# jarek1992/raytracer_project

Measured on AMD Instinct MI355X. Metric: Msamples/sec (rays·bounces), higher is better.
Workload: dtype f64

## Files before the change

raytracer_project_amd/csrc/zr_commit.cpp:

```cpp
#include "zr_host_internal.h"
#include "zr_flatten.h"

namespace {

template <class F>
int each_prim_array(zr_scene* s, Flattener& fl, F&& f) {
    int rc;
    if ((rc = f(s->d_spheres, fl.spheres, ZR_PRIM_SPHERE, ZR_SPHERE_DOUBLES)) || (rc = f(s->d_sphere_mat, fl.sphere_mat, ZR_PRIM_SPHERE, 1)) ||
        (rc = f(s->d_tri_v, fl.tri_v, ZR_PRIM_TRIANGLE, ZR_TRI_STRIDE)) || (rc = f(s->d_tri_s, fl.tri_s, ZR_PRIM_TRIANGLE, ZR_TRI_SHADE_DOUBLES)) ||
        (rc = f(s->d_cubes, fl.cubes, ZR_PRIM_CUBE, ZR_CUBE_DOUBLES)) || (rc = f(s->d_cube_mat, fl.cube_mat, ZR_PRIM_CUBE, 1)) ||
        (rc = f(s->d_pcubes, fl.pcubes, ZR_KIND_PCUBE, ZR_PCUBE_STRIDE)) || (rc = f(s->d_pcube_mat, fl.pcube_mat, ZR_KIND_PCUBE, 1)) ||
        (rc = f(s->d_media, fl.media, ZR_PRIM_MEDIUM, 1)) || (rc = f(s->d_wrapped, fl.wrapped, ZR_KIND_WRAPPED, 1))) return rc;
    return ZR_OK;
}

int commit_host(zr_scene* s, std::shared_ptr<const CommitPlan> plan, PhaseTimer& ph, CommitSummary& cs, std::shared_ptr<HostBuild>& staging) {
    auto hb = std::make_shared<HostBuild>();
    int rc = build_host_tree(*s, plan, ph, *hb);
    if (rc) return rc;
    Flattener& fl = *hb->fl;
    int up_rc = ZR_OK;
    std::string up_err;
    std::thread uploader;
    const int device = s->ctx ? s->ctx->device : 0;
// ... 233 lines not shown
    d.cubes = s->d_cubes.p; d.cube_mat = s->d_cube_mat.p;
    d.pcubes = s->d_pcubes.p; d.pcube_mat = s->d_pcube_mat.p;
    d.media = s->d_media.p; d.wrapped = s->d_wrapped.p; d.insts = s->d_insts.p; d.ops = s->d_ops.p;
    d.mats = s->d_mats.p; d.texs = s->d_texs.p; d.texels = s->d_texels.p;
    d.n_mats = (uint32_t)s->materials.size();
    d.mat_kinds = 0;
    for (const zr_material& m : s->materials) d.mat_kinds |= 1u << m.kind;
    d.root = cs.root;
    s->leaf_objects = 0;
    for (int k = 0; k < 8; k++) { d.leaf_cnt[k] = plan.cnt[k]; s->leaf_objects += plan.cnt[k]; }
    s->fused_ok = false;
    if (s->leaf_objects > 0 && s->leaf_objects <= ZR_FUSED_OBJECTS && plan.cnt[ZR_KIND_INSTANCE] == 0) {
        zr::FusedObjs fo{};
        auto take = [&](uint32_t kind, const double* d_src, size_t stride, size_t doubles) -> int {
            for (uint32_t i = 0; i < plan.cnt[kind]; i++) {
                fo.kind[fo.n] = kind; fo.index[fo.n] = i;
                HIP_OK(hipMemcpy(fo.rec[fo.n], d_src + (size_t)i * stride, doubles * sizeof(double), hipMemcpyDeviceToHost));
                fo.n++;
            }
            return ZR_OK;
        };
        if ((rc = take(ZR_PRIM_SPHERE, s->d_spheres.p, ZR_SPHERE_DOUBLES, ZR_SPHERE_DOUBLES)) || (rc = take(ZR_PRIM_TRIANGLE, s->d_tri_v.p, ZR_TRI_STRIDE, 9)) ||
            (rc = take(ZR_PRIM_CUBE, s->d_cubes.p, ZR_CUBE_DOUBLES, ZR_CUBE_DOUBLES)) || (rc = take(ZR_KIND_PCUBE, s->d_pcubes.p, ZR_PCUBE_STRIDE, ZR_PCUBE_STRIDE))) return rc;
        std::vector<zr::DMedium> hm(plan.cnt[ZR_PRIM_MEDIUM]);
        if (!hm.empty()) HIP_OK(hipMemcpy(hm.data(), s->d_media.p, hm.size() * sizeof(zr::DMedium), hipMemcpyDeviceToHost));
        for (uint32_t i = 0; i < hm.size(); i++) {
            if (hm[i].chain_count != 0) continue;
            fo.kind[fo.n] = ZR_PRIM_MEDIUM; fo.index[fo.n] = i;
            const bool sph = hm[i].btype == ZR_PRIM_SPHERE;
            HIP_OK(hipMemcpy(fo.rec[fo.n], sph ? s->d_spheres.p + (size_t)hm[i].bindex * ZR_SPHERE_DOUBLES : s->d_cubes.p + (size_t)hm[i].bindex * ZR_CUBE_DOUBLES, (sph ? ZR_SPHERE_DOUBLES : ZR_CUBE_DOUBLES) * sizeof(double), hipMemcpyDeviceToHost));
            fo.rec[fo.n][6] = hm[i].neg_inv_density;
            const uint64_t idb = hm[i].id, tb = hm[i].btype;
            std::memcpy(&fo.rec[fo.n][7], &idb, 8); std::memcpy(&fo.rec[fo.n][8], &tb, 8);
            fo.n++;
        }
        bool scaled = false;
        for (uint32_t i = 0; i < fo.n; i++) if (fo.kind[i] == ZR_KIND_PCUBE && fo.rec[i][15] != 0.0) scaled = true;
        s->fused = fo; s->fused_ok = !scaled;
    }
    {
        if (z[ZR_KIND_INSTANCE]) s->leaf_level = 3;
        else if (z[ZR_KIND_WRAPPED] || !cs.plain_media) s->leaf_level = 2;
        else if (z[ZR_PRIM_CUBE] || z[ZR_KIND_PCUBE] || z[ZR_PRIM_MEDIUM]) s->leaf_level = 1;
        else s->leaf_level = 0;
        const int force = (int)env_double("ZR_EXTEND_LEVEL", -1);
        if (force > s->leaf_level && force <= 3) s->leaf_level = force;
        bool lean = s->leaf_level == 0 && env_double("ZR_SHADE_LEAN", 1) != 0;
        for (const zr_material& m : s->materials) {
            if (m.kind != ZR_MAT_LAMBERTIAN && m.kind != ZR_MAT_METAL && m.kind != ZR_MAT_DIELECTRIC && m.kind != ZR_MAT_LIGHT) lean = false;
            if (m.bump_tex != ZR_NO_TEXTURE) lean = false;
            if (m.kind != ZR_MAT_DIELECTRIC && (m.tex >= s->textures.size() || s->textures[m.tex].kind != ZR_TEX_SOLID)) lean = false;
        }
        d.shade_lean = lean ? 1u : 0u;
        d.shade_escape = lean && env_double("ZR_SHADE_ESCAPE", 1) != 0 ? 1u : 0u;
    }
    s->stack_demand = cs.stack_demand;
    if (std::getenv("ZR_QUANT_STATS")) std::fprintf(stderr, "[zr] 4-wide tree: depth %d, worst-case traversal stack %u entries\n", cs.quad_depth, s->stack_demand);
    s->stats[0] = cs.n_pairs; s->stats[1] = (uint64_t)cs.max_depth; s->stats[2] = plan.objs.size();
    s->stats[3] = cs.n_pairs * sizeof(zr::NodePair) + cs.n_quads * sizeof(zr::NodeQ) + (z[ZR_PRIM_SPHERE] * ZR_SPHERE_DOUBLES + z[ZR_PRIM_TRIANGLE] * (ZR_TRI_STRIDE + ZR_TRI_SHADE_DOUBLES) + z[ZR_PRIM_CUBE] * ZR_CUBE_DOUBLES +
                   z[ZR_KIND_PCUBE] * ZR_PCUBE_STRIDE) * sizeof(double) + (z[ZR_PRIM_SPHERE] + z[ZR_PRIM_CUBE]) * sizeof(uint32_t) + s->texels.size();
    s->builder = cs.builder;
    if (std::getenv("ZR_COMMIT_HASH")) {
        (void)hipDeviceSynchronize();
        auto fnv = [](const void* dev, size_t bytes) -> unsigned long long {
            std::vector<unsigned char> h(bytes);
            unsigned long long x = 1469598103934665603ull;
            if (bytes && hipMemcpy(h.data(), dev, bytes, hipMemcpyDeviceToHost) == hipSuccess) for (unsigned char b : h) { x ^= b; x *= 1099511628211ull; }
            return x;
        };
        std::fprintf(stderr, "[zr] commit hash (%s): quads %016llx (%zu), pairs %016llx (%zu)\n", cs.builder, fnv(s->d_quads.p, cs.n_quads * sizeof(zr::NodeQ)), cs.n_quads,
                     fnv(s->d_nodes.p, cs.n_pairs * sizeof(zr::NodePair)), cs.n_pairs);
    }
    s->committed = true;
    if (s->borrowed) {
        s->spheres.drop(); s->sphere_mat.drop(); s->tri_v.drop(); s->tri_n.drop(); s->tri_mat.drop(); s->cubes.drop(); s->cube_mat.drop();
        s->media.drop(); s->ops.drop(); s->objects.drop(); s->texels.drop(); s->objects_set = false; s->borrowed = false; s->released = true;
    }
    return ZR_OK;
}

}

extern "C" {

zr_scene* zr_scene_create(zr_ctx* c) {
    if (!c) { fail(ZR_E_INVALID, "null context"); return nullptr; }
    zr_scene* s = new zr_scene();
    s->ctx = c; s->device = c->device;
    return s;
}
void zr_scene_destroy(zr_scene* s) {
    if (!s) return;
    (void)hipSetDevice(s->device);
    delete s;
}

enum { SET_SPHERES = 1, SET_TRIANGLES = 2, SET_CUBES = 4, SET_MEDIA = 8, SET_OPS = 16, SET_OBJECTS = 32, SET_ALL_GEOMETRY = 63 };
#define CHECK_SCENE(s) do { if (!(s)) return fail(ZR_E_INVALID, "null scene"); (s)->committed = false; } while (0)
#define GEOMETRY_SET(s, bit) do { if ((s)->released) { (s)->reset_mask |= (bit); if (((s)->reset_mask & SET_ALL_GEOMETRY) == SET_ALL_GEOMETRY) { (s)->released = false; (s)->reset_mask = 0; } } } while (0)

int zr_scene_set_spheres(zr_scene* s, const double* p, const uint32_t* mat, size_t n) {
    CHECK_SCENE(s);
    if (n && (!p || !mat)) return fail(ZR_E_INVALID, "null sphere arrays");
    s->spheres.copy(p, n * 4); s->sphere_mat.copy(mat, n);
    GEOMETRY_SET(s, SET_SPHERES);
    return ZR_OK;
}
// ... 127 lines not shown
```

raytracer_project_amd/csrc/zr_device.h:

```cpp
#pragma once

#include <hip/hip_runtime.h>
#include <stdint.h>

#include "../../include/zr_capi.h"
#include "../../include/zr_rng.h"

#include "zr_device_types.h"

namespace zr {

struct V3 { double x, y, z; };
__device__ __forceinline__ V3 mk(double x, double y, double z) { V3 r; r.x = x; r.y = y; r.z = z; return r; }
__device__ __forceinline__ V3 operator+(V3 a, V3 b) { return mk(a.x + b.x, a.y + b.y, a.z + b.z); }
__device__ __forceinline__ V3 operator-(V3 a, V3 b) { return mk(a.x - b.x, a.y - b.y, a.z - b.z); }
__device__ __forceinline__ V3 operator-(V3 a) { return mk(-a.x, -a.y, -a.z); }
__device__ __forceinline__ V3 operator*(V3 a, V3 b) { return mk(a.x * b.x, a.y * b.y, a.z * b.z); }
__device__ __forceinline__ V3 operator*(double t, V3 v) { return mk(t * v.x, t * v.y, t * v.z); }
__device__ __forceinline__ V3 operator*(V3 v, double t) { return mk(t * v.x, t * v.y, t * v.z); }
__device__ __forceinline__ V3 vdiv(V3 v, double t) { double r = 1 / t; return mk(r * v.x, r * v.y, r * v.z); }
__device__ __forceinline__ double dot(V3 a, V3 b) { return a.x * b.x + a.y * b.y + a.z * b.z; }
__device__ __forceinline__ V3 cross(V3 a, V3 b) { return mk(a.y * b.z - a.z * b.y, a.z * b.x - a.x * b.z, a.x * b.y - a.y * b.x); }
__device__ __forceinline__ double len2(V3 a) { return a.x * a.x + a.y * a.y + a.z * a.z; }
__device__ __forceinline__ double len(V3 a) { return sqrt(len2(a)); }
// ... 783 lines not shown
    em = mk(0, 0, 0);
    if (rec.mat >= sc.n_mats) return false;
    const zr_material& m = sc.mats[rec.mat];
    const uint32_t kind = m.kind;
    if (kind == ZR_MAT_LIGHT) { em = lean_color(sc, m.tex); return false; }
    V3 ruv = mk(0, 0, 0);
    if (kind == ZR_MAT_LAMBERTIAN || kind == ZR_MAT_METAL) ruv = random_unit_vector(g);
    V3 ud = mk(0, 0, 0);
    if (kind == ZR_MAT_METAL || kind == ZR_MAT_DIELECTRIC) ud = unit(rin.d);
    if (kind == ZR_MAT_LAMBERTIAN) {
        V3 dir = rec.n + ruv;
        if (fabs(dir.x) < 1e-8 && fabs(dir.y) < 1e-8 && fabs(dir.z) < 1e-8) dir = rec.n;
        out.o = rec.p + (rec.n * 0.0001);
        out.d = dir;
        att = lean_color(sc, m.tex);
        return true;
    }
    if (kind == ZR_MAT_METAL) {
        V3 refl = reflect(ud, rec.n);
        V3 dir = unit(refl + (m.param * ruv));
        out.o = rec.p + (0.0001 * rec.n);
        out.d = dir;
        att = lean_color(sc, m.tex);
        return dot(dir, rec.n) > 0;
    }
    if (kind == ZR_MAT_DIELECTRIC) {
        att = mk(m.tint[0], m.tint[1], m.tint[2]);
        double ri = rec.front ? (1.0 / m.param) : m.param;
        double ct = fmin(dot(-ud, rec.n), 1.0);
        double st = sqrt(1.0 - ct * ct);
        bool refl = ri * st > 1.0;
        if (!refl) {
            double r0 = (1 - ri) / (1 + ri);
            r0 = r0 * r0;
            double rf = r0 + (1 - r0) * pow5(1 - ct);
            refl = rf > g.next();
        }
        V3 dir;
        if (refl) dir = reflect(ud, rec.n);
        else {
            double c2 = fmin(dot(-ud, rec.n), 1.0);
            V3 perp = ri * (ud + c2 * rec.n);
            V3 par = (-sqrt(fabs(1.0 - len2(perp)))) * rec.n;
            dir = perp + par;
        }
        V3 off = (dot(dir, rec.n) > 0) ? (0.0001 * rec.n) : (-0.0001 * rec.n);
        out.o = rec.p + off;
        out.d = dir;
        return true;
    }
    return false;
}

__device__ inline V3 background(const DScene& sc, const DEnv& env, V3 rd) {
    if (env.mode == ZR_ENV_SOLID_COLOR) return mk(env.solid[0], env.solid[1], env.solid[2]);
    V3 ud = unit(rd);
    if (env.mode == ZR_ENV_HDR_MAP) {
        if (env.hdr_tex == ZR_NO_TEXTURE) return mk(0, 0, 0);
        V3 d = ud;
        double x1 = env.cy * d.x + env.sy * d.z;
        double z1 = -env.sy * d.x + env.cy * d.z;
        d = mk(x1, d.y, z1);
        double y2 = env.cp * d.y - env.sp * d.z;
        double z2 = env.sp * d.y + env.cp * d.z;
        d = mk(d.x, y2, z2);
        double x3 = env.cr * d.x - env.sr * d.y;
        double y3 = env.sr * d.x + env.cr * d.y;
        d = mk(x3, y3, d.z);
        const double PI = 3.14159265358979323846;
        const zr_texture& t = sc.texs[env.hdr_tex];
        if (t.kind == ZR_TEX_IMAGE_F32 && t.width > 0 && t.height > 0 && t.width <= 16384 && t.height <= 16384) {
            const float xf = (float)d.x, yf = (float)d.y, zf = (float)d.z;
            const float PIf = 3.14159265358979323846f;
            const float fi = (atan2f(zf, xf) + PIf) * (0.15915494309189535f * (float)t.width);
            const float fj = acosf(fminf(fmaxf(yf, -1.0f), 1.0f)) * (0.3183098861837907f * (float)t.height);
            const float ri = fi - floorf(fi), rj = fj - floorf(fj);
            const float guard = 0.02f;
            if (fabsf(yf) < 0.999f && ri > guard && ri < 1.0f - guard && rj > guard && rj < 1.0f - guard && fi > guard &&
                fi < (float)t.width - guard) {
                const int i = (int)fi, j = (int)fj;
                const float* px = (const float*)(sc.texels + t.texel_offset) + ((size_t)j * t.width + i) * 3;
                return mk((double)px[0], (double)px[1], (double)px[2]) * env.intensity;
            }
        }
        double phi = atan2(d.z, d.x) + PI;
        double theta = acos(clampd(d.y, -1.0, 1.0));
        return tex_value(sc, env.hdr_tex, phi / (2 * PI), theta / PI, mk(0, 0, 0)) * env.intensity;
    }
    V3 hor = mk(env.horizon[0], env.horizon[1], env.horizon[2]);
    V3 zen = mk(env.zenith[0], env.zenith[1], env.zenith[2]);
    V3 sun = mk(env.sun[0], env.sun[1], env.sun[2]);
    double a = ud.y;
    V3 sky;
    if (a > 0.0) sky = (1.0 - a) * hor + a * zen; else sky = hor * 0.1;
    V3 fin = (sky * env.sky_scale) * env.sky_exposure;
    double focus = dot(ud, sun);
    if (env.sun_on && focus > env.sun_thr) {
        double x = clampd((focus - env.sun_thr) / ((env.sun_thr + 0.0002) - env.sun_thr), 0.0, 1.0);
        double alpha = x * x * (3 - 2 * x);
        fin = fin + mk(env.sun_add[0], env.sun_add[1], env.sun_add[2]) * alpha;
    }
    return fin;
}

__device__ inline Ray camera_ray(const DCamera& cam, int i, int j, Rng& g) {
    double ox = g.next() - 0.5;
    double oy = g.next() - 0.5;
    V3 ps = ld3(cam.pixel00) + ((i + ox) * ld3(cam.du)) + ((j + oy) * ld3(cam.dv));
    V3 org = ld3(cam.center);
    if (cam.defocus) {
        double px, py;
        for (;;) {
            px = g.range(-1, 1);
            py = g.range(-1, 1);
            if (px * px + py * py + 0.0 * 0.0 < 1) break;
        }
        org = ld3(cam.center) + (px * ld3(cam.disk_u)) + (py * ld3(cam.disk_v));
    }
    Ray r; r.o = org; r.d = ps - org;
    return r;
}

}
```

raytracer_project_amd/csrc/zr_device_types.h:

```cpp
#pragma once
#include <stdint.h>
#include "../../include/zr_capi.h"

#define ZR_KIND_WRAPPED 4u
#define ZR_KIND_PCUBE 5u
#define ZR_KIND_INSTANCE 6u
#ifndef ZR_TRI_STRIDE
#define ZR_TRI_STRIDE 9
#endif
#define ZR_SPHERE_DOUBLES 4
#define ZR_CUBE_DOUBLES 6
#define ZR_TRI_SHADE_DOUBLES 20
#define ZR_STACK_DEPTH 48
#define ZR_MAX_CHAIN 8

namespace zr {

struct alignas(64) NodePair {
    float lo[2][3];
    float hi[2][3];
    uint32_t child[2];
    uint32_t meta[2];
};
static_assert(sizeof(NodePair) == 64, "NodePair must be 64 bytes");

#define ZR_PCUBE_STRIDE 16
#define ZR_REF_LEAF 0x80000000u
#define ZR_REF_EMPTY 0xFFFFFFFFu
struct alignas(64) NodeQ {
    float origin[3];
    float scale[3];
    uint32_t q[6];
    uint32_t ref[4];
};
static_assert(sizeof(NodeQ) == 64, "NodeQ must be 64 bytes");
struct NodeF {
    float lox[4], loy[4], loz[4], hix[4], hiy[4], hiz[4];
    uint32_t ref[4];
};

struct DMedium {
    uint32_t btype, bindex, chain_first, chain_count;
    uint32_t mat, id;
    double neg_inv_density;
};
struct DWrapped { uint32_t type, index, chain_first, chain_count; };
struct DInstance { uint32_t chain_first, chain_count, root , pad_ ; };

struct DScene {
    const NodePair* nodes;
    const NodeQ* quads;
    const double* spheres;
    const uint32_t* sphere_mat;
    const double* tri_v;
    const double* tri_s;
    const double* cubes;
    const uint32_t* cube_mat;
    const double* pcubes;
    const uint32_t* pcube_mat;
    const DMedium* media;
    const DWrapped* wrapped;
    const DInstance* insts;
    const zr_xform_op* ops;
    const zr_material* mats;
    const zr_texture* texs;
    const unsigned char* texels;
    uint32_t n_mats;
    uint32_t mat_kinds;
    uint32_t shade_lean;
    uint32_t leaf_cnt[8];
    NodeF root;
    uint32_t shade_escape;
};

struct DCamera {
    double center[3], pixel00[3], du[3], dv[3], disk_u[3], disk_v[3];
    int32_t W, H, spp, max_depth;
    int32_t defocus;
    int32_t pad_;
};

struct DEnv {
    uint32_t mode, hdr_tex;
    double solid[3];
    double cy, sy, cp, sp, cr, sr;
    double intensity;
    double sun[3];
    double horizon[3], zenith[3];
    double sky_scale, sky_exposure;
    double sun_thr;
    double sun_add[3];
    int32_t sun_on, pad_;
};

}
```

raytracer_project_amd/csrc/zr_stream.hip:

```cpp
#include "zr_device.h"
#include "zr_launch.h"

namespace zr {

#ifndef ST_EXT_WAVES
#define ST_EXT_WAVES 4
#endif
#ifndef ST_CHUNK
#define ST_CHUNK 256
#endif
#ifndef ST_SHADE_WAVES
#define ST_SHADE_WAVES 4
#endif
#ifndef ST_EXT_WAVES_LEAN
#define ST_EXT_WAVES_LEAN 6
#endif
#ifndef ST_EXT_WAVES_MID
#define ST_EXT_WAVES_MID 4
#endif
#ifndef ST_FETCH_MIN
#define ST_FETCH_MIN 16
#endif
#define ST_SHARDS 64
#ifndef ST_LDS_STACK
#define ST_LDS_STACK 12
#endif

enum { F_FIRST = 1u << 16, F_ACTIVE = 1u << 17, F_L0 = 1u << 18,
       F_LZERO = 1u << 19 , F_BONE = 1u << 20  };

struct SEntry { uint32_t node; float tn; };

enum { SF_RAY = 0, SF_HIT_T = 6, SF_HIT_KI = 7, SF_BETA = 8, SF_L = 11, SF_ATT0 = 14, SF_SUM = 17, SF_KEY = 20,
       SF_MA = 21 , SF_MB = 22 , SF_N = 24 };

enum { CTL_COMPACT = 4,
       CTL_SHARD0 = 16, CTL_STRIDE = 32,
       CTL_SH_UNITS = 0,
       CTL_SH_CHUNK = 8,
       CTL_SH_ACTIVE = 16 };

struct StreamBuf {
    double* pool;
    const uint32_t* pixels;
    double* samples;
    unsigned int* ctl;
    unsigned int* uctl;
    uint32_t P, spp, n_units, n_pix;
    uint32_t unit0;
    uint32_t unit_base;
    uint32_t unit_chunk;
    uint32_t shard_k0;
    uint32_t sample0;
    uint2* kend;
    unsigned char* cls;
    unsigned long long* cpart;
    __device__ __forceinline__ double* cell(int f, uint32_t slot) const { return pool + ((size_t)(slot >> 6) * SF_N + f) * 64 + (slot & 63u); }
    __device__ __forceinline__ double ld(int f, uint32_t slot) const { return *cell(f, slot); }
    __device__ __forceinline__ void st(int f, uint32_t slot, double v) const { *cell(f, slot) = v; }
    __device__ __forceinline__ uint2 ld2(int f, uint32_t slot) const { return *reinterpret_cast<const uint2*>(cell(f, slot)); }
    __device__ __forceinline__ void st2(int f, uint32_t slot, uint2 v) const { *reinterpret_cast<uint2*>(cell(f, slot)) = v; }
    __device__ __forceinline__ V3 ld3(int f, uint32_t slot) const { return mk(ld(f, slot), ld(f + 1, slot), ld(f + 2, slot)); }
    __device__ __forceinline__ void st3(int f, uint32_t slot, V3 v) const { st(f, slot, v.x); st(f + 1, slot, v.y); st(f + 2, slot, v.z); }
};

struct SlotAt {
    const char* base; uint32_t off;
    __device__ __forceinline__ const char* at(int f) const { return base + (off + (uint32_t)f * 512u); }
    __device__ __forceinline__ double ld(int f) const { return *reinterpret_cast<const double*>(at(f)); }
    __device__ __forceinline__ void st(int f, double v) const { *reinterpret_cast<double*>(const_cast<char*>(at(f))) = v; }
    __device__ __forceinline__ uint2 ld2(int f) const { return *reinterpret_cast<const uint2*>(at(f)); }
    __device__ __forceinline__ void st2(int f, uint2 v) const { *reinterpret_cast<uint2*>(const_cast<char*>(at(f))) = v; }
    __device__ __forceinline__ V3 ld3(int f) const { return mk(ld(f), ld(f + 1), ld(f + 2)); }
    __device__ __forceinline__ void st3(int f, V3 v) const { st(f, v.x); st(f + 1, v.y); st(f + 2, v.z); }
};
__device__ __forceinline__ SlotAt slot_at(const StreamBuf& B, uint32_t block, uint32_t src) {
    SlotAt a;
    a.base = reinterpret_cast<const char*>(B.pool) + (size_t)block * (size_t)(4 * SF_N * 512);
    a.off = (src >> 6) * (uint32_t)(SF_N * 512) + (src & 63u) * 8u;
    return a;
}


__host__ __device__ inline unsigned long long st_unit_of(uint32_t G, uint32_t unit_base, uint32_t shard, unsigned long long k) {
    if (G == 0) return (unsigned long long)unit_base + k * ST_SHARDS + shard;
    const uint32_t k32 = (uint32_t)k, q = k32 / G, r = k32 - q * G;
    const uint32_t pos = (shard & 7u) * (ST_SHARDS / 8u) + (shard >> 3);
    return ((unsigned long long)q * ST_SHARDS + pos) * G + r;
}
__host__ __device__ inline unsigned long long st_first_unit(uint32_t G, uint32_t g) {
    if (G == 0) return g;
    const uint32_t c = g >> 8;
    return st_unit_of(G, 0, c % ST_SHARDS, (unsigned long long)(c / ST_SHARDS) * 256u + (g & 255u));
}

__device__ inline void begin_sample(const StreamBuf& B, const DCamera& cam, uint64_t seed, const SlotAt& S, uint32_t unit, uint32_t& c_samp) {
    const uint32_t pix_i = unit / B.spp, sample = unit - pix_i * B.spp + B.sample0;
    const uint32_t pk = B.pixels[pix_i];
    const int px = (int)(pk & 0xFFFFu), py = (int)(pk >> 16);
    Rng g; g.key = zr_stream_key(seed, (uint64_t)py * (uint64_t)cam.W + (uint64_t)px, (uint64_t)sample); g.k = 0; g.bounce = 0;
    Ray r = camera_ray(cam, px, py, g);
    S.st3(SF_RAY, r.o); S.st3(SF_RAY + 3, r.d);
    S.st(SF_KEY, __longlong_as_double((long long)g.key));
    uint2 ma; ma.x = (uint32_t)g.k; ma.y = F_FIRST | F_ACTIVE;
    uint2 mb; mb.x = unit; mb.y = 0;
    S.st2(SF_MA, ma); S.st2(SF_MB, mb);
    c_samp++;
}

template <bool COUNT>
__global__ __launch_bounds__(256) void stream_init(StreamBuf B, DCamera cam, uint64_t seed, unsigned long long* __restrict__ gctr) {
    const uint32_t slot = blockIdx.x * 256 + threadIdx.x;
    if (slot >= B.P) return;
    uint32_t c_samp = 0;
    const unsigned long long u0 = st_first_unit(B.unit_chunk, B.unit0 + slot);
    const SlotAt S = slot_at(B, blockIdx.x, threadIdx.x);
    if (u0 < (unsigned long long)B.n_units) begin_sample(B, cam, seed, S, (uint32_t)u0, c_samp);
    else { uint2 z; z.x = 0; z.y = 0; S.st2(SF_MA, z); }
    if (COUNT && c_samp) atomicAdd(&gctr[CTR_SAMPLES], (unsigned long long)c_samp);
}

enum { X_IDLE = 0, X_NODE = 1, X_LEAF = 2 };
#define X_LEAF_BIT ZR_REF_LEAF

__device__ __forceinline__ void cswap(float& ta, uint32_t& ra, float& tb, uint32_t& rb) {
    const bool sw = tb < ta;
    const float t0 = sw ? tb : ta, t1 = sw ? ta : tb;
    const uint32_t r0 = sw ? rb : ra, r1 = sw ? ra : rb;
    ta = t0; tb = t1; ra = r0; rb = r1;
}

#ifndef ST_EXT_GROUP
#define ST_EXT_GROUP 1
#endif
template <bool COUNT, int LEVEL>
__global__ __launch_bounds__(64 * ST_EXT_GROUP, LEVEL >= 2 ? ST_EXT_WAVES : (LEVEL == 1 ? ST_EXT_WAVES_MID : ST_EXT_WAVES_LEAN)) void stream_extend(DScene sc, StreamBuf B, SEntry* __restrict__ overflow,
                                                                  uint32_t ovf_levels, unsigned long long* __restrict__ gctr) {
    __shared__ SEntry lstack[ST_EXT_GROUP * ST_LDS_STACK * 64];
    const int lane = threadIdx.x & 63;
    const uint32_t wave_id = blockIdx.x * ST_EXT_GROUP + (threadIdx.x >> 6);
    const int lbase = (int)(threadIdx.x >> 6) * ST_LDS_STACK * 64 + lane;
    const unsigned long long lt_mask = (1ull << lane) - 1ull;
    SEntry* gstack = overflow + (size_t)wave_id * ovf_levels * 64 + lane;
    const double INF = __builtin_huge_val();
    const float INFf = __builtin_huge_valf();
    const uint32_t NONE = 0xFFFFFFFFu;

    int st = X_IDLE;
    uint32_t slot = 0;
    Ray ray; ray.o = mk(0, 0, 0); ray.d = mk(0, 0, 1);
    float idx_ = 0, idy_ = 0, idz_ = 0;
    float cnx = 0, cny = 0, cnz = 0, cfx = 0, cfy = 0, cfz = 0;
    double tbest = INF;
    float tbest_f = INFf;
    uint32_t kbest = NONE, ibest = 0;
    uint32_t inst_cur = 0;
    uint32_t cur = 0;
    uint32_t pend_i = 0;
    int sp = 0;
// ... 193 lines not shown
                }
                bool h;
                if (LEVEL == 3 && lkind == ZR_KIND_INSTANCE) {
                    const DInstance in = sc.insts[prim];
                    ZR_PUSH(ZR_REF_LEAF | (7u << 28), -INFf)
                    ray = chain_ray(sc, in.chain_first, in.chain_count, ray);
                    ZR_RAY_CONSTANTS()
                    inst_cur = prim + 1u;
                    cur = in.pad_; pend_i = 0; st = X_NODE;
                } else if (LEVEL == 3 && lkind == 7u) {
                    ray.o = B.ld3(SF_RAY, slot); ray.d = B.ld3(SF_RAY + 3, slot);
                    ZR_RAY_CONSTANTS()
                    inst_cur = 0;
                    ZR_POP_NEXT()
                } else {
                if (LEVEL == 1) {
                    if (lkind == ZR_KIND_PCUBE) h = pcube_t(sc.pcubes + (size_t)prim * ZR_PCUBE_STRIDE, ray, 0.001, tbest, t);
                    else if (lkind == ZR_PRIM_CUBE) h = cube_t(sc.cubes + (size_t)prim * 6, ray, 0.001, tbest, t);
                    else h = medium_plain_t(sc, prim, ray, 0.001, tbest, g, t);
                } else h = object_t(sc, lkind, prim, ray, 0.001, tbest, g, t);
                if (h) { tbest = t; tbest_f = __double2float_ru(t); kbest = lkind; ibest = prim; }
                tested = true;
                }
            }
            if (tested) {
                pend_i++;
                if (pend_i > ((cur >> 24) & 0xFu)) { ZR_POP_NEXT() }
            }
        }
    }
    if (iter >= iter_cap && lane == 0) atomicAdd(&B.ctl[CTL_CAPPED], 1u);
#ifdef ZR_WAVE_PROFILE
    if (!COUNT && lane == 0) {
        atomicAdd(&gctr[CTR_PROF_WAVE_TICKS], wall_clock64() - t_begin); atomicAdd(&gctr[CTR_PROF_WAVES], 1ull);
        for (int k = 0; k < 3; k++) { atomicAdd(&gctr[CTR_PROF_EXECS + 2 * k], p_exec[k]); atomicAdd(&gctr[CTR_PROF_LANES + 2 * k], p_lanes[k]); }
        for (int k = 0; k < CTR_HIST_WORDS; k++) if (p_hist[threadIdx.x >> 6][k]) atomicAdd(&gctr[CTR_HIST + k], (unsigned long long)p_hist[threadIdx.x >> 6][k]);
    }
#endif
    if (COUNT) {
        atomicAdd(&gctr[CTR_SEGMENTS], (unsigned long long)c_seg);
        atomicAdd(&gctr[CTR_NODES], (unsigned long long)c_nodes);
        atomicAdd(&gctr[CTR_SPHERES], (unsigned long long)c_sph);
        atomicAdd(&gctr[CTR_TRIANGLES], (unsigned long long)c_tri);
        atomicAdd(&gctr[CTR_CUBES], (unsigned long long)c_cube);
        atomicAdd(&gctr[CTR_MEDIA], (unsigned long long)c_med);
        atomicAdd(&gctr[CTR_HITS], (unsigned long long)c_hits);
        if (lane == 0) for (int k = 0; k < 2; k++) { atomicAdd(&gctr[CTR_NODE_EXECS + 2 * k], s_exec[k]); atomicAdd(&gctr[CTR_NODE_LANES + 2 * k], s_lanes[k]); }
    }
}

#ifndef ST_SHADE_WAVES_LEAN
#define ST_SHADE_WAVES_LEAN 6
#endif
template <bool COUNT, int MODE, bool LEAN = false>
__global__ __launch_bounds__(256, LEAN ? ST_SHADE_WAVES_LEAN : ST_SHADE_WAVES) void stream_shade(DScene sc, DCamera cam, DEnv env, uint64_t seed, StreamBuf B,
                                                    unsigned long long* __restrict__ gctr) {
    const uint32_t slot0 = blockIdx.x * 256 + threadIdx.x;
    if (slot0 < ST_SHARDS) B.ctl[CTL_SHARD0 + CTL_STRIDE * slot0 + CTL_SH_CHUNK] = 0;
    __shared__ unsigned long long s_cnt[4];
    if (MODE != 0 && threadIdx.x < 4) s_cnt[threadIdx.x] = 0;
    __shared__ unsigned int wave_cls[4][8];
    __shared__ uint4 x_mk[256];
    __shared__ unsigned char x_src[256];
    uint32_t src;
    uint2 m, ki;
    {
        uint2 m0; m0.x = 0; m0.y = 0;
        uint2 k0; k0.x = 0xFFFFFFFFu; k0.y = 0;
        if (slot0 < B.P) { const SlotAt S0 = slot_at(B, blockIdx.x, threadIdx.x); m0 = S0.ld2(SF_MA); k0 = S0.ld2(SF_HIT_KI); }
        uint32_t cls = 7;
        if (m0.y & F_ACTIVE) {
            if (k0.x == 0xFFFFFFFFu) cls = 6;
            else {
                cls = 0;
                if (sc.mat_kinds & (sc.mat_kinds - 1u)) {
                    const uint32_t mat = object_material(sc, k0.x, k0.y);
                    cls = mat < sc.n_mats ? sc.mats[mat].kind : 5u;
                    if (cls > 5u) cls = 5u;
                }
            }
        }
        const int w = threadIdx.x >> 6, wl = threadIdx.x & 63;
        const unsigned long long below = (1ull << wl) - 1ull;
        unsigned int my_rank = 0;
#pragma unroll
        for (uint32_t c = 0; c < 8; c++) {
            const unsigned long long bm = __ballot(cls == c);
            if (wl == 0) wave_cls[w][c] = (unsigned int)__popcll(bm);
            if (cls == c) my_rank = (unsigned int)__popcll(bm & below);
        }
        __syncthreads();
        unsigned int base = 0;
        for (uint32_t c = 0; c < 8; c++)
            for (int k = 0; k < 4; k++)
                if (c < cls || (c == cls && k < w)) base += wave_cls[k][c];
        uint4 mk4; mk4.x = m0.x; mk4.y = m0.y; mk4.z = k0.x; mk4.w = k0.y;
        x_mk[base + my_rank] = mk4;
        x_src[base + my_rank] = (unsigned char)threadIdx.x;
        __syncthreads();
        mk4 = x_mk[threadIdx.x];
        src = x_src[threadIdx.x];
        m.x = mk4.x; m.y = mk4.y; ki.x = mk4.z; ki.y = mk4.w;
    }
    const SlotAt S = slot_at(B, blockIdx.x, src);
    bool active_after = false, want_unit = false;
    uint32_t c_samp = 0, c_seg2 = 0, c_hit2 = 0, c_esc = 0, c_esc_nodes = 0, c_seen = 0; unsigned long long c_draws = 0;
// ... 94 lines not shown
                                if (g.next() > p) stop = true; else beta = beta * (1 / p);
                            }
                        }
                    }
                    if (!stop) { b_inner++; if (b_inner >= depth_inner) stop = true; }
                    if (stop) {
                        if (!have_L) L = load_L();
                        if (MODE == 2) { const double luma = 0.2126 * len(L); if (luma > 2.0) L = L * (2.0 / luma); }
                        contrib = S.ld3(SF_ATT0) * L; ended = true;
                    } else if (esc) {
                        att0_now = S.ld3(SF_ATT0); beta_now = beta;
                        if (have_L) { L_now = L; have_L_now = true; }
                    } else {
                        if (have_L) { S.st3(SF_L, L); keep_lzero = 0; }
                        S.st3(SF_BETA, beta);
                    }
                }
                if (!ended && esc) {
                    escaped = true; miss_first = false;
                    ray = nr;
                    if (COUNT) { c_esc++; c_esc_nodes += esc_nodes; }
                } else if (!ended) {
                    S.st3(SF_RAY, nr.o); S.st3(SF_RAY + 3, nr.d);
                    if (has_add) S.st3(SF_SUM, add_now);
                    m.x = (uint32_t)g.k;
                    m.y = (g.bounce & 0xFFu) | ((uint32_t)b_inner << 8) | F_ACTIVE | (first ? (has_add ? F_L0 : 0u) : (m.y & F_L0)) |
                          (first ? (F_LZERO | F_BONE) : keep_lzero);
                    S.st2(SF_MA, m);
                    active_after = true;
                }
            }
            if (ESC && (ki.x == NONE || escaped)) ZR_MISS_STAGE()
#undef ZR_MISS_STAGE
            if (ended) {
                V3 rad = contrib;
                if (has_add) rad = add_now + rad;
                else if (MODE != 2 && !first && (m.y & F_L0)) rad = S.ld3(SF_SUM) + rad;
                const uint2 mb = mb_now;
                const uint32_t unit = mb.x;
                if (MODE != 2 || !no_output) {
                    double* pp = B.samples + (size_t)unit * 3;
                    pp[0] = rad.x; pp[1] = rad.y; pp[2] = rad.z;
                }
                if (MODE == 1) { uint2 ke; ke.x = (uint32_t)g.k; ke.y = g.bounce; B.kend[unit] = ke; }
                if (MODE == 2 && !no_output) B.cls[unit] = (unsigned char)mb.y;
                if (COUNT) {
                    if (MODE != 2) c_draws += g.k;
                    else if (!(first && ki.x == NONE)) c_draws += g.k - B.kend[unit].x;
                }
                want_unit = true;
            }
        }
    }
    {
        const unsigned long long wm = __ballot(want_unit);
        if (wm != 0ull) {
            const uint32_t shard = blockIdx.x % ST_SHARDS;
            const int wl = threadIdx.x & 63;
            uint32_t k0 = 0;
            if (wl == (int)__builtin_ctzll(wm)) k0 = atomicAdd(&B.uctl[CTL_STRIDE * shard + CTL_SH_UNITS], (unsigned int)__popcll(wm));
            k0 = __shfl(k0, (int)__builtin_ctzll(wm), 64);
            if (want_unit) {
                const unsigned long long k = (unsigned long long)k0 + (unsigned long long)__popcll(wm & ((1ull << wl) - 1ull));
                const unsigned long long u = st_unit_of(B.unit_chunk, B.unit_base, shard, (unsigned long long)B.shard_k0 + k);
                if (u < (unsigned long long)B.n_units) { begin_sample(B, cam, seed, S, (uint32_t)u, c_samp); active_after = true; }
                else { uint2 z; z.x = 0; z.y = 0; S.st2(SF_MA, z); }
            }
        }
    }
    const unsigned long long am = __ballot(active_after);
    if ((threadIdx.x & 63) == 0 && am != 0ull) atomicAdd(&B.ctl[CTL_SHARD0 + CTL_STRIDE * (blockIdx.x % ST_SHARDS) + CTL_SH_ACTIVE], (unsigned int)__popcll(am));
    if (COUNT && MODE == 0) {
        if (c_samp) atomicAdd(&gctr[CTR_SAMPLES], (unsigned long long)c_samp);
        if (c_draws) atomicAdd(&gctr[CTR_DRAWS], c_draws);
        if (c_seen) atomicAdd(&gctr[CTR_SHADE_LANES], (unsigned long long)c_seen);
        if (c_esc) {
            atomicAdd(&gctr[CTR_SEGMENTS], (unsigned long long)c_esc); atomicAdd(&gctr[CTR_ESCAPED], (unsigned long long)c_esc);
            atomicAdd(&gctr[CTR_NODES], (unsigned long long)c_esc_nodes);
        }
    }
    if (MODE != 0) {
        if (c_samp) atomicAdd(&s_cnt[0], (unsigned long long)c_samp);
        if (c_seg2) atomicAdd(&s_cnt[1], (unsigned long long)c_seg2);
        if (c_hit2) atomicAdd(&s_cnt[2], (unsigned long long)c_hit2);
        if (c_draws) atomicAdd(&s_cnt[3], c_draws);
        __syncthreads();
        if (threadIdx.x < 4 && s_cnt[threadIdx.x]) B.cpart[(size_t)blockIdx.x * 4 + threadIdx.x] += s_cnt[threadIdx.x];
    }
}

#ifndef ST_FUSED_CHUNK
#define ST_FUSED_CHUNK 256
#endif
#ifndef ST_FUSED_WAVES
#define ST_FUSED_WAVES 2
#endif
struct FusedBuf {
    const uint32_t* pixels; double* samples; unsigned int* uctl;
    uint32_t spp, n_units;
    uint32_t sample0;
    uint32_t chunk_lo, chunk_hi;
};
__device__ __forceinline__ bool medium_rec_t(const double* q, const Ray& r, double tmin, double tmax, const Rng& g, double& t) {
    double t1, t2;
    const double inf = __builtin_huge_val();
    const uint32_t btype = (uint32_t)__double_as_longlong(q[8]);
    if (btype == ZR_PRIM_SPHERE) {
        if (!sphere_t(q, r, -inf, inf, t1)) return false;
        if (!sphere_t(q, r, t1 + 0.0001, inf, t2)) return false;
    } else {
        if (!cube_t(q, r, -inf, inf, t1)) return false;
        if (!cube_t(q, r, t1 + 0.0001, inf, t2)) return false;
    }
    if (t1 < tmin) t1 = tmin;
    if (t2 > tmax) t2 = tmax;
    if (t1 >= t2) return false;
    if (t1 < 0) t1 = 0;
    const double rl = len(r.d);
    const double inside = (t2 - t1) * rl;
// ... 266 lines not shown
    uint2 ma; ma.x = 0; ma.y = 0;
    if (slot < n) {
        B.st3(SF_RAY, slot, ld3(rays + (size_t)slot * 6)); B.st3(SF_RAY + 3, slot, ld3(rays + (size_t)slot * 6 + 3));
        B.st(SF_KEY, slot, __longlong_as_double((long long)zr_stream_key(seed, pixel, (uint64_t)slot)));
        ma.y = (bounce & 0xFFu) | F_ACTIVE;
    }
    B.st2(SF_MA, slot, ma);
}

__global__ __launch_bounds__(256) void stream_hits_out(DScene sc, StreamBuf B, uint32_t n, zr_hit* __restrict__ out) {
    const uint32_t slot = blockIdx.x * 256 + threadIdx.x;
    if (slot >= n) return;
    const uint2 ki = B.ld2(SF_HIT_KI, slot);
    zr_hit o;
    if (ki.x != 0xFFFFFFFFu) {
        Ray r; r.o = B.ld3(SF_RAY, slot); r.d = B.ld3(SF_RAY + 3, slot);
        Rec rec;
        object_rec(sc, ki.x, ki.y, r, B.ld(SF_HIT_T, slot), rec, true);
        o.p[0] = rec.p.x; o.p[1] = rec.p.y; o.p[2] = rec.p.z;
        o.normal[0] = rec.n.x; o.normal[1] = rec.n.y; o.normal[2] = rec.n.z;
        o.tangent[0] = rec.tan.x; o.tangent[1] = rec.tan.y; o.tangent[2] = rec.tan.z;
        o.bitangent[0] = rec.bit.x; o.bitangent[1] = rec.bit.y; o.bitangent[2] = rec.bit.z;
        o.t = rec.t; o.u = rec.u; o.v = rec.v; o.mat = rec.mat; o.front_face = rec.front ? 1u : 0u;
    } else {
        for (int c = 0; c < 3; c++) { o.p[c] = 0; o.normal[c] = 0; o.tangent[c] = 0; o.bitangent[c] = 0; }
        o.t = 0; o.u = 0; o.v = 0; o.mat = 0xFFFFFFFFu; o.front_face = 0;
    }
    out[slot] = o;
}

size_t stream_ctl_words() { return CTL_SHARD0 + CTL_STRIDE * ST_SHARDS; }
uint32_t stream_overflow_levels(uint32_t stack_demand) { return stack_demand > ST_LDS_STACK ? stack_demand - ST_LDS_STACK : 1u; }
size_t stream_overflow_bytes(int blocks, uint32_t levels) { return (size_t)blocks * levels * 64 * sizeof(SEntry); }

int stream_extend_blocks() {
    int dev = 0, cus = 256, per_cu = 2;
    if (hipGetDevice(&dev) == hipSuccess) {
        hipDeviceProp_t p;
        if (hipGetDeviceProperties(&p, dev) == hipSuccess) cus = p.multiProcessorCount;
    }
    int lean = 0;
    if (hipOccupancyMaxActiveBlocksPerMultiprocessor(&per_cu, stream_extend<false, 2>, 64 * ST_EXT_GROUP, 0) != hipSuccess || per_cu < 1) per_cu = 2;
    if (hipOccupancyMaxActiveBlocksPerMultiprocessor(&lean, stream_extend<false, 0>, 64 * ST_EXT_GROUP, 0) == hipSuccess && lean > per_cu) per_cu = lean;
    if (std::getenv("ZR_COMMIT_STATS")) std::fprintf(stderr, "[zr] EXTEND workgroups per CU: %d (lean build %d) x %d waves\n", per_cu, lean, ST_EXT_GROUP);
    return cus * per_cu * ST_EXT_GROUP;
}

size_t stream_pool_bytes(uint32_t P) { return ((size_t)(P + 63) / 64) * SF_N * 64 * sizeof(double); }

static StreamBuf make_buf(void* pool, uint32_t P, uint32_t spp, uint32_t n_units, uint32_t n_pix, const uint32_t* pixels, double* samples,
                          unsigned int* ctl, unsigned int* uctl, uint32_t unit0, uint32_t unit_base) {
    StreamBuf B;
    B.pool = (double*)pool; B.pixels = pixels; B.samples = samples; B.ctl = ctl; B.uctl = uctl;
    B.P = P; B.spp = spp; B.n_units = n_units; B.n_pix = n_pix; B.unit0 = unit0; B.unit_base = unit_base; B.unit_chunk = 0; B.shard_k0 = 0; B.sample0 = 0;
    B.kend = nullptr; B.cls = nullptr; B.cpart = nullptr;
    return B;
}

template <bool COUNT>
static void launch_extend(const DScene& sc, const StreamBuf& B, void* overflow, uint32_t ovf_levels, int blocks, unsigned long long* gctr, int level, hipStream_t st) {
    const dim3 grid((blocks + ST_EXT_GROUP - 1) / ST_EXT_GROUP), group(64 * ST_EXT_GROUP);
    if (level >= 3) hipLaunchKernelGGL((stream_extend<COUNT, 3>), grid, group, 0, st, sc, B, (SEntry*)overflow, ovf_levels, gctr);
    else if (level == 2) hipLaunchKernelGGL((stream_extend<COUNT, 2>), grid, group, 0, st, sc, B, (SEntry*)overflow, ovf_levels, gctr);
    else if (level == 1) hipLaunchKernelGGL((stream_extend<COUNT, 1>), grid, group, 0, st, sc, B, (SEntry*)overflow, ovf_levels, gctr);
    else hipLaunchKernelGGL((stream_extend<COUNT, 0>), grid, group, 0, st, sc, B, (SEntry*)overflow, ovf_levels, gctr);
}

hipError_t stream_render(const DScene& sc, const StreamJob& job, int leaf_level) {
    const StreamFrame& F = job.frame; const StreamContext& X = job.ctx; const StreamHooks& H = job.hooks;
    const DCamera& cam = *F.cam; const DEnv& env = *F.env;
    const uint32_t P = job.pool.P, unit_chunk = job.pool.unit_chunk, n_pix = F.n_pix;
    const int mode = job.split.mode;
    const uint32_t n_units = n_pix * F.spp;
    const size_t W = stream_ctl_words();
    int K = X.n_pools < 1 ? 1 : (X.n_pools > ST_MAX_POOLS ? ST_MAX_POOLS : X.n_pools);
    while (K > 1 && P / K < 64u * 1024u) K--;
    const uint32_t pool_round = unit_chunk ? ST_SHARDS * 256u : 64u;
    if (unit_chunk && P % pool_round != 0) return hipErrorInvalidValue;
    while (K > 1 && P / K < pool_round) K--;
    StreamBuf Q[ST_MAX_POOLS];
    void* ov[ST_MAX_POOLS];
    unsigned int* uctl = X.ctl + (size_t)ST_MAX_POOLS * W;
    const unsigned int* h_units = X.h_active + (size_t)ST_MAX_POOLS * W;
    {
        uint32_t first = 0;
        unsigned char* base = (unsigned char*)job.pool.slots;
        for (int k = 0; k < K; k++) {
            uint32_t Pk = k == K - 1 ? P - first : (P / K + pool_round - 1) / pool_round * pool_round;
            Q[k] = make_buf(base, Pk, F.spp, n_units, n_pix, F.pixels, F.samples, X.ctl + (size_t)k * W, uctl, first, P);
            Q[k].unit_chunk = unit_chunk; Q[k].shard_k0 = unit_chunk ? P / ST_SHARDS : 0u; Q[k].sample0 = F.sample0;
            Q[k].kend = (uint2*)job.split.kend; Q[k].cls = (unsigned char*)job.split.cls;
            Q[k].cpart = job.split.cpart ? job.split.cpart + ((size_t)first / 256 + (size_t)k) * 4 : nullptr;
            ov[k] = (unsigned char*)X.overflow + (size_t)k * stream_overflow_bytes(X.extend_blocks, X.ovf_levels);
            base += stream_pool_bytes(Pk);
            first += Pk;
        }
    }
    hipError_t e;
    hipStream_t stream = X.streams[0];
    if ((e = hipMemsetAsync(X.ctl, 0, (ST_MAX_POOLS + 1) * W * sizeof(unsigned int), stream)) != hipSuccess) return e;
    const size_t cpart_blocks = (size_t)P / 256 + ST_MAX_POOLS + 1;
    if (job.split.cpart && (e = hipMemsetAsync(job.split.cpart, 0, cpart_blocks * 4 * sizeof(unsigned long long), stream)) != hipSuccess) return e;
    auto init = [&](const StreamBuf& B, hipStream_t st) {
        if (H.timer) H.timer->begin(st, 0);
        if (F.count) hipLaunchKernelGGL(stream_init<true>, dim3((B.P + 255) / 256), dim3(256), 0, st, B, cam, F.seed, X.gctr);
        else hipLaunchKernelGGL(stream_init<false>, dim3((B.P + 255) / 256), dim3(256), 0, st, B, cam, F.seed, X.gctr);
        if (H.timer) H.timer->end(st, 0);
    };
    auto extend = [&](const StreamBuf& B, void* o, hipStream_t st) {
        const int eb = (int)((B.P + 63) / 64 < (uint32_t)X.extend_blocks ? (B.P + 63) / 64 : (uint32_t)X.extend_blocks);
        if (H.timer) H.timer->begin(st, 1);
        if (F.count) launch_extend<true>(sc, B, o, X.ovf_levels, eb, X.gctr, leaf_level, st); else launch_extend<false>(sc, B, o, X.ovf_levels, eb, X.gctr, leaf_level, st);
        if (H.timer) H.timer->end(st, 1);
    };
    static const unsigned shade_pad = std::getenv("ZR_SHADE_LDS_PAD") ? (unsigned)std::atoi(std::getenv("ZR_SHADE_LDS_PAD")) : 0u;
    auto shade = [&](const StreamBuf& B, hipStream_t st) {
        if (H.timer) H.timer->begin(st, 2);
        const dim3 sg((B.P + 255) / 256), sb(256);
        if (sc.shade_lean && mode == 0) {
            if (F.count) hipLaunchKernelGGL((stream_shade<true, 0, true>), sg, sb, 0, st, sc, cam, env, F.seed, B, X.gctr);
            else hipLaunchKernelGGL((stream_shade<false, 0, true>), sg, sb, shade_pad, st, sc, cam, env, F.seed, B, X.gctr);
        }
        else if (shade_pad && mode == 0 && !F.count) hipLaunchKernelGGL((stream_shade<false, 0>), sg, sb, shade_pad, st, sc, cam, env, F.seed, B, X.gctr);
        else if (mode == 1) hipLaunchKernelGGL((stream_shade<true, 1>), sg, sb, 0, st, sc, cam, env, F.seed, B, X.gctr);
        else if (mode == 2) hipLaunchKernelGGL((stream_shade<true, 2>), sg, sb, 0, st, sc, cam, env, F.seed, B, X.gctr);
        else if (F.count) hipLaunchKernelGGL((stream_shade<true, 0>), sg, sb, 0, st, sc, cam, env, F.seed, B, X.gctr);
        else hipLaunchKernelGGL((stream_shade<false, 0>), sg, sb, 0, st, sc, cam, env, F.seed, B, X.gctr);
        if (H.timer) H.timer->end(st, 2);
    };
    init(Q[0], stream);
    for (int k = 1; k < K; k++) {
        extend(Q[k - 1], ov[k - 1], X.streams[k - 1]);
        if ((e = hipEventRecord(X.event, X.streams[k - 1])) != hipSuccess) return e;
        if ((e = hipStreamWaitEvent(X.streams[k], X.event, 0)) != hipSuccess) return e;
        init(Q[k], X.streams[k]);
        shade(Q[k - 1], X.streams[k - 1]);
    }
    int rounds = K > 1 ? 1 : 0;
    int check_every = H.progress ? 2 : 8;
    bool cancelled = false, drained = false, capped = false;
    for (;;) {
        for (int r = 0; r < check_every; r++) {
            for (int k = K - 1; k >= 0; k--) { extend(Q[k], ov[k], X.streams[k]); shade(Q[k], X.streams[k]); }
// ... 147 lines not shown
```

Baseline: 6956.

## Regenerate camera samples in lean shade and resolve provably escaping rays directly

In the lean shade kernel (MODE 0), a fresh camera sample is now tested with ray_escapes against the scene root when it is generated. If the ray provably misses all geometry, its background colour is written straight to the sample buffer and another unit is fetched in a loop, so such rays skip a full extend/shade round trip through the stream pool. Kernel arguments are reloaded from the kernarg segment pointer, presumably to limit register pressure. The change adds extra divergence and atomics per wave. regen_max defaults to 0, which leaves the loop unbounded, and the escape level now defaults to 2, so the new path runs by default.

```diff
diff --git a/raytracer_project_amd/csrc/zr_commit.cpp b/raytracer_project_amd/csrc/zr_commit.cpp
--- a/raytracer_project_amd/csrc/zr_commit.cpp
+++ b/raytracer_project_amd/csrc/zr_commit.cpp
@@ -309,7 +309,9 @@
             if (m.kind != ZR_MAT_DIELECTRIC && (m.tex >= s->textures.size() || s->textures[m.tex].kind != ZR_TEX_SOLID)) lean = false;
         }
         d.shade_lean = lean ? 1u : 0u;
-        d.shade_escape = lean && env_double("ZR_SHADE_ESCAPE", 1) != 0 ? 1u : 0u;
+        const double esc_level = env_double("ZR_SHADE_ESCAPE", 2), regen_max = env_double("ZR_SHADE_REGEN_MAX", ZR_SHADE_REGEN_MAX_DEFAULT);
+        d.shade_escape = (uint16_t)(lean && esc_level >= 1 ? (esc_level >= 2 ? 2 : 1) : 0);
+        d.regen_max = (uint16_t)(regen_max >= 1 ? std::min(regen_max, 65535.0) : 0);
     }
     s->stack_demand = cs.stack_demand;
     if (std::getenv("ZR_QUANT_STATS")) std::fprintf(stderr, "[zr] 4-wide tree: depth %d, worst-case traversal stack %u entries\n", cs.quad_depth, s->stack_demand);
diff --git a/raytracer_project_amd/csrc/zr_device.h b/raytracer_project_amd/csrc/zr_device.h
--- a/raytracer_project_amd/csrc/zr_device.h
+++ b/raytracer_project_amd/csrc/zr_device.h
@@ -859,9 +859,14 @@
     return false;
 }
 
-__device__ inline V3 background(const DScene& sc, const DEnv& env, V3 rd) {
+template <bool DIRECT = false>
+__device__ inline V3 background(const DScene& sc, const DEnv& env, V3 rd, bool* direct_ok = nullptr) {
     if (env.mode == ZR_ENV_SOLID_COLOR) return mk(env.solid[0], env.solid[1], env.solid[2]);
-    V3 ud = unit(rd);
+    V3 ud;
+    if (DIRECT) {
+        const double l = sqrt(__builtin_fma(rd.z, rd.z, __builtin_fma(rd.x, rd.x, rd.y * rd.y)));
+        ud = l < 1e-8 ? mk(0, 0, 0) : vdiv(rd, l);
+    } else ud = unit(rd);
     if (env.mode == ZR_ENV_HDR_MAP) {
         if (env.hdr_tex == ZR_NO_TEXTURE) return mk(0, 0, 0);
         V3 d = ud;
@@ -890,6 +895,7 @@
                 return mk((double)px[0], (double)px[1], (double)px[2]) * env.intensity;
             }
         }
+        if (DIRECT) { *direct_ok = false; return mk(0, 0, 0); }
         double phi = atan2(d.z, d.x) + PI;
         double theta = acos(clampd(d.y, -1.0, 1.0));
         return tex_value(sc, env.hdr_tex, phi / (2 * PI), theta / PI, mk(0, 0, 0)) * env.intensity;
@@ -899,9 +905,12 @@
     V3 sun = mk(env.sun[0], env.sun[1], env.sun[2]);
     double a = ud.y;
     V3 sky;
-    if (a > 0.0) sky = (1.0 - a) * hor + a * zen; else sky = hor * 0.1;
+    if (a > 0.0) {
+        if (DIRECT) { const double b = 1.0 - a; sky = mk(__builtin_fma(zen.x, a, b * hor.x), __builtin_fma(zen.y, a, b * hor.y), __builtin_fma(zen.z, a, b * hor.z)); }
+        else sky = (1.0 - a) * hor + a * zen;
+    } else sky = hor * 0.1;
     V3 fin = (sky * env.sky_scale) * env.sky_exposure;
-    double focus = dot(ud, sun);
+    double focus = DIRECT ? __builtin_fma(ud.z, sun.z, __builtin_fma(ud.x, sun.x, ud.y * sun.y)) : dot(ud, sun);
     if (env.sun_on && focus > env.sun_thr) {
         double x = clampd((focus - env.sun_thr) / ((env.sun_thr + 0.0002) - env.sun_thr), 0.0, 1.0);
         double alpha = x * x * (3 - 2 * x);
diff --git a/raytracer_project_amd/csrc/zr_device_types.h b/raytracer_project_amd/csrc/zr_device_types.h
--- a/raytracer_project_amd/csrc/zr_device_types.h
+++ b/raytracer_project_amd/csrc/zr_device_types.h
@@ -13,6 +13,9 @@
 #define ZR_TRI_SHADE_DOUBLES 20
 #define ZR_STACK_DEPTH 48
 #define ZR_MAX_CHAIN 8
+#ifndef ZR_SHADE_REGEN_MAX_DEFAULT
+#define ZR_SHADE_REGEN_MAX_DEFAULT 0
+#endif
 
 namespace zr {
 
@@ -70,7 +73,8 @@
     uint32_t shade_lean;
     uint32_t leaf_cnt[8];
     NodeF root;
-    uint32_t shade_escape;
+    uint16_t shade_escape;
+    uint16_t regen_max;
 };
 
 struct DCamera {
diff --git a/raytracer_project_amd/csrc/zr_stream.hip b/raytracer_project_amd/csrc/zr_stream.hip
--- a/raytracer_project_amd/csrc/zr_stream.hip
+++ b/raytracer_project_amd/csrc/zr_stream.hip
@@ -52,6 +52,7 @@
     uint32_t unit_chunk;
     uint32_t shard_k0;
     uint32_t sample0;
+    uint32_t regen_max;
     uint2* kend;
     unsigned char* cls;
     unsigned long long* cpart;
@@ -94,17 +95,24 @@
     return st_unit_of(G, 0, c % ST_SHARDS, (unsigned long long)(c / ST_SHARDS) * 256u + (g & 255u));
 }
 
-__device__ inline void begin_sample(const StreamBuf& B, const DCamera& cam, uint64_t seed, const SlotAt& S, uint32_t unit, uint32_t& c_samp) {
+__device__ __forceinline__ Ray make_sample(const StreamBuf& B, const DCamera& cam, uint64_t seed, uint32_t unit, Rng& g) {
     const uint32_t pix_i = unit / B.spp, sample = unit - pix_i * B.spp + B.sample0;
     const uint32_t pk = B.pixels[pix_i];
     const int px = (int)(pk & 0xFFFFu), py = (int)(pk >> 16);
-    Rng g; g.key = zr_stream_key(seed, (uint64_t)py * (uint64_t)cam.W + (uint64_t)px, (uint64_t)sample); g.k = 0; g.bounce = 0;
-    Ray r = camera_ray(cam, px, py, g);
+    g.key = zr_stream_key(seed, (uint64_t)py * (uint64_t)cam.W + (uint64_t)px, (uint64_t)sample); g.k = 0; g.bounce = 0;
+    return camera_ray(cam, px, py, g);
+}
+__device__ __forceinline__ void store_sample(const SlotAt& S, const Ray& r, const Rng& g, uint32_t unit) {
     S.st3(SF_RAY, r.o); S.st3(SF_RAY + 3, r.d);
     S.st(SF_KEY, __longlong_as_double((long long)g.key));
     uint2 ma; ma.x = (uint32_t)g.k; ma.y = F_FIRST | F_ACTIVE;
     uint2 mb; mb.x = unit; mb.y = 0;
     S.st2(SF_MA, ma); S.st2(SF_MB, mb);
+}
+__device__ inline void begin_sample(const StreamBuf& B, const DCamera& cam, uint64_t seed, const SlotAt& S, uint32_t unit, uint32_t& c_samp) {
+    Rng g;
+    const Ray r = make_sample(B, cam, seed, unit, g);
+    store_sample(S, r, g, unit);
     c_samp++;
 }
 
@@ -404,6 +412,7 @@
 #ifndef ST_SHADE_WAVES_LEAN
 #define ST_SHADE_WAVES_LEAN 6
 #endif
+struct ShadeArgs { DScene sc; DCamera cam; DEnv env; uint64_t seed; StreamBuf B; unsigned long long* gctr; };
 template <bool COUNT, int MODE, bool LEAN = false>
 __global__ __launch_bounds__(256, LEAN ? ST_SHADE_WAVES_LEAN : ST_SHADE_WAVES) void stream_shade(DScene sc, DCamera cam, DEnv env, uint64_t seed, StreamBuf B,
                                                     unsigned long long* __restrict__ gctr) {
@@ -604,7 +613,8 @@
             }
         }
     }
-    {
+    constexpr bool REGEN = LEAN && MODE == 0;
+    if (!REGEN) {
         const unsigned long long wm = __ballot(want_unit);
         if (wm != 0ull) {
             const uint32_t shard = blockIdx.x % ST_SHARDS;
@@ -617,6 +627,52 @@
                 const unsigned long long u = st_unit_of(B.unit_chunk, B.unit_base, shard, (unsigned long long)B.shard_k0 + k);
                 if (u < (unsigned long long)B.n_units) { begin_sample(B, cam, seed, S, (uint32_t)u, c_samp); active_after = true; }
                 else { uint2 z; z.x = 0; z.y = 0; S.st2(SF_MA, z); }
+            }
+        }
+    } else {
+        typedef const __attribute__((address_space(4))) ShadeArgs* KernArgs;
+        KernArgs A4 = (KernArgs)__builtin_amdgcn_kernarg_segment_ptr();
+        uint32_t regen_left = 0xFFFFFFFFu;
+        const uint32_t shard = blockIdx.x % ST_SHARDS;
+        const int wl = threadIdx.x & 63;
+#pragma nounroll
+        for (uint32_t pass = 0;; pass++) {
+            const unsigned long long wm = __ballot(want_unit);
+            if (wm == 0ull) break;
+            asm volatile("" : "+s"(A4));
+            const ShadeArgs* A = (const ShadeArgs*)A4;
+            const StreamBuf& Bk = A->B;
+            if (pass == 0 && Bk.regen_max) regen_left = Bk.regen_max;
+            uint32_t k0 = 0;
+            if (wl == (int)__builtin_ctzll(wm)) k0 = atomicAdd(&Bk.uctl[CTL_STRIDE * shard + CTL_SH_UNITS], (unsigned int)__popcll(wm));
+            k0 = __shfl(k0, (int)__builtin_ctzll(wm), 64);
+            bool proven = false;
+            Ray r2; r2.o = mk(0, 0, 0); r2.d = mk(0, 0, 1);
+            Rng g2; g2.key = 0; g2.k = 0; g2.bounce = 0;
+            uint32_t u2 = 0, esc_nodes = 0;
+            if (want_unit) {
+                want_unit = false;
+                const unsigned long long k = (unsigned long long)k0 + (unsigned long long)__popcll(wm & ((1ull << wl) - 1ull));
+                const unsigned long long u = st_unit_of(Bk.unit_chunk, Bk.unit_base, shard, (unsigned long long)Bk.shard_k0 + k);
+                if (u < (unsigned long long)Bk.n_units) {
+                    u2 = (uint32_t)u;
+                    r2 = make_sample(Bk, A->cam, A->seed, u2, g2);
+                    c_samp++;
+                    proven = A->sc.shade_escape >= 2 && regen_left != 0u && ray_escapes(r2, A->sc.root, A->sc.spheres, esc_nodes);
+                    if (!proven) { store_sample(S, r2, g2, u2); active_after = true; }
+                } else { uint2 z; z.x = 0; z.y = 0; S.st2(SF_MA, z); }
+            }
+            if (__ballot(proven) == 0ull) break;
+            if (proven) {
+                bool direct = true;
+                const V3 bg = background<true>(A->sc, A->env, r2.d, &direct);
+                if (direct) {
+                    double* pp = Bk.samples + (size_t)u2 * 3;
+                    pp[0] = bg.x; pp[1] = bg.y; pp[2] = bg.z;
+                    if (COUNT) { c_draws += g2.k; c_esc++; c_esc_nodes += esc_nodes; }
+                    regen_left--;
+                    want_unit = true;
+                } else { store_sample(S, r2, g2, u2); active_after = true; }
             }
         }
     }
@@ -989,7 +1045,7 @@
                           unsigned int* ctl, unsigned int* uctl, uint32_t unit0, uint32_t unit_base) {
     StreamBuf B;
     B.pool = (double*)pool; B.pixels = pixels; B.samples = samples; B.ctl = ctl; B.uctl = uctl;
-    B.P = P; B.spp = spp; B.n_units = n_units; B.n_pix = n_pix; B.unit0 = unit0; B.unit_base = unit_base; B.unit_chunk = 0; B.shard_k0 = 0; B.sample0 = 0;
+    B.P = P; B.spp = spp; B.n_units = n_units; B.n_pix = n_pix; B.unit0 = unit0; B.unit_base = unit_base; B.unit_chunk = 0; B.shard_k0 = 0; B.sample0 = 0; B.regen_max = 0;
     B.kend = nullptr; B.cls = nullptr; B.cpart = nullptr;
     return B;
 }
@@ -1025,7 +1081,7 @@
         for (int k = 0; k < K; k++) {
             uint32_t Pk = k == K - 1 ? P - first : (P / K + pool_round - 1) / pool_round * pool_round;
             Q[k] = make_buf(base, Pk, F.spp, n_units, n_pix, F.pixels, F.samples, X.ctl + (size_t)k * W, uctl, first, P);
-            Q[k].unit_chunk = unit_chunk; Q[k].shard_k0 = unit_chunk ? P / ST_SHARDS : 0u; Q[k].sample0 = F.sample0;
+            Q[k].unit_chunk = unit_chunk; Q[k].shard_k0 = unit_chunk ? P / ST_SHARDS : 0u; Q[k].sample0 = F.sample0; Q[k].regen_max = sc.regen_max;
             Q[k].kend = (uint2*)job.split.kend; Q[k].cls = (unsigned char*)job.split.cls;
             Q[k].cpart = job.split.cpart ? job.split.cpart + ((size_t)first / 256 + (size_t)k) * 4 : nullptr;
             ov[k] = (unsigned char*)X.overflow + (size_t)k * stream_overflow_bytes(X.extend_blocks, X.ovf_levels);
```

New measurement: 6464. 0.929x the previous value.
